# cnuns/Com-MARL

Measured on AMD Instinct MI355X. Metric: env-steps/sec (whole node), PredatorPrey M=10 N=4, 4096 envs at 1/2/4/8 GPUs, higher is better.
Workload: dtype f32

## Files before the change

### com-marl_amd/_lib.py

```python
import ctypes as C
import os

HERE = os.path.dirname(os.path.abspath(__file__))
LIB_PATH = os.environ.get("COMMARL_LIB") or os.path.join(HERE, "libcommarl_hip.so")

CM_PP, CM_CO = 0, 1
PACK_F32, PACK_F16, PACK_WAVE, PACK_CHECK, PACK_ALL = 1, 2, 4, 8, 15
CHANNELS = {"FC": 0, "FL": 1, "IID": 2, "GE": 3}
RNG_PHILOX, RNG_TAPE = 0, 1
ENT_ADD, ENT_SOFTPLUS, ENT_STOP_GRAD = 1, 2, 4
EPI_COLS, SUM_COLS = 9, 12
COMM_COLS, EPC_COLS = 4, 4
ATTN_COLS, EPA_COLS = 6, 6
LISTEN_COLS, EPL_COLS = 6, 6


class EnvCfg(C.Structure):
    _fields_ = [(n, C.c_int32) for n in (
        "scenario", "n_envs", "n_agents", "n_preys", "grid", "rsen", "load", "max_steps", "max_path_length",
        "n_hops", "rcom", "channel", "obst_hard", "add_clock", "rng_mode", "env_id_offset")] + [
        ("ploss", C.c_float), ("pgb", C.c_float), ("pbg", C.c_float), ("ge_flags", C.c_int32)] + [
        (n, C.c_double) for n in ("capture_reward", "step_cost", "move_cost", "penalty", "lazy_penalty",
                                  "revisit_penalty", "final_reward")] + [("seed", C.c_uint64)]

# ... 197 lines not shown
    "cm_comm_means": (C.c_int, [C.c_int32, C.c_int32, C.c_void_p, C.c_void_p, C.c_void_p]),
    "cm_episode_curves": (C.c_int, [C.c_int32, C.c_int32, C.c_int32, C.c_int32, C.c_void_p, C.c_void_p, C.c_void_p, C.c_void_p,
                                    C.c_void_p, C.c_int32, C.c_int32, C.c_int32, C.c_void_p, C.c_void_p]),
    "cm_curve_means": (C.c_int, [C.c_int32, C.c_int32, C.c_int32, C.c_int32, C.c_int32, C.c_void_p, C.c_void_p, C.c_void_p]),
    "cm_comm_curves": (C.c_int, [C.c_int32, C.c_int32, C.c_int32, C.c_int32, C.c_void_p, C.c_void_p, C.c_int32, C.c_int32,
                                 C.c_int32, C.c_void_p, C.c_void_p]),
    "cm_comm_curve_means": (C.c_int, [C.c_int32, C.c_int32, C.c_int32, C.c_int32, C.c_int32, C.c_void_p, C.c_void_p, C.c_void_p]),
    "cm_attn_stats": (C.c_int, [C.c_int32, C.c_int32, C.c_int32, C.c_void_p, C.c_int64, C.c_void_p, C.c_int64, C.c_void_p, C.c_int64,
                                C.c_void_p, C.c_void_p]),
    "cm_episode_attn": (C.c_int, [C.c_int32, C.c_int32, C.c_int32, C.c_int32, C.c_void_p, C.c_void_p, C.c_int32, C.c_int32,
                                  C.c_int32, C.c_int32, C.c_void_p, C.c_void_p]),
    "cm_attn_means": (C.c_int, [C.c_int32, C.c_int32, C.c_void_p, C.c_void_p, C.c_void_p]),
    "cm_attn_curves": (C.c_int, [C.c_int32, C.c_int32, C.c_int32, C.c_int32, C.c_void_p, C.c_void_p, C.c_int32, C.c_int32,
                                 C.c_int32, C.c_void_p, C.c_void_p]),
    "cm_attn_curve_means": (C.c_int, [C.c_int32, C.c_int32, C.c_int32, C.c_int32, C.c_int32, C.c_void_p, C.c_void_p, C.c_void_p]),
    "cm_listen_stats": (C.c_int, [C.c_int32, C.c_int32, C.c_int32, C.c_void_p, C.c_int64, C.c_void_p, C.c_int64, C.c_void_p, C.c_int64,
                                  C.c_void_p, C.c_void_p]),
    "cm_episode_listen": (C.c_int, [C.c_int32, C.c_int32, C.c_int32, C.c_void_p, C.c_void_p, C.c_int32, C.c_int32, C.c_int32,
                                    C.c_int32, C.c_void_p, C.c_void_p]),
    "cm_listen_means": (C.c_int, [C.c_int32, C.c_int32, C.c_void_p, C.c_void_p, C.c_void_p]),
    "cm_listen_curves": (C.c_int, [C.c_int32, C.c_int32, C.c_int32, C.c_void_p, C.c_void_p, C.c_int32, C.c_int32, C.c_int32,
                                   C.c_void_p, C.c_void_p]),
    "cm_listen_curve_means": (C.c_int, [C.c_int32, C.c_int32, C.c_int32, C.c_int32, C.c_void_p, C.c_void_p, C.c_void_p]),
    "cm_chunk_tail": (C.c_int, [C.c_void_p, C.c_uint32, C.c_void_p, C.c_void_p, C.c_size_t, C.c_void_p, C.c_void_p,
                                C.c_size_t, C.c_void_p, C.c_void_p, C.c_size_t, C.c_void_p]),
    "cm_linear_act_forward": (C.c_int, [C.c_int64, C.c_int32, C.c_int32, C.c_void_p, C.c_void_p, C.c_int32, C.c_void_p,
                                        C.c_int32, C.c_void_p, C.c_void_p]),
    "cm_linear_act_backward": (C.c_int, [C.c_int64, C.c_int32, C.c_int32, C.c_void_p, C.c_void_p, C.c_int32, C.c_void_p,
                                         C.c_void_p, C.c_void_p, C.c_void_p, C.c_void_p, C.c_void_p, C.c_void_p]),
    "cm_linear_act_backward_ex": (C.c_int, [C.c_int64, C.c_int32, C.c_int32, C.c_void_p, C.c_void_p, C.c_int32, C.c_void_p,
                                            C.c_void_p, C.c_void_p, C.c_int32, C.c_void_p, C.c_void_p, C.c_void_p, C.c_void_p]),
    "cm_encoder_backward": (C.c_int, [C.c_int64, C.c_int32, C.c_void_p, C.c_void_p, C.c_void_p, C.c_void_p, C.c_void_p, C.c_void_p,
                                      C.c_void_p, C.c_void_p, C.c_void_p, C.c_void_p, C.c_void_p]),
    "cm_multi_copy_t": (C.c_int, [C.c_int32, C.c_void_p, C.c_void_p, C.c_void_p, C.c_void_p, C.c_void_p, C.c_void_p]),
    "cm_multi_adam_step": (C.c_int, [C.c_int32, C.c_void_p, C.c_void_p, C.c_void_p, C.c_void_p, C.c_void_p, C.c_void_p,
                                     C.c_float, C.c_float, C.c_float, C.c_float, C.c_float, C.c_int32, C.c_void_p]),
    "cm_gauss_nll_forward": (C.c_int, [C.c_int64, C.c_int32, C.c_void_p, C.c_void_p, C.c_void_p, C.c_float, C.c_int32, C.c_void_p, C.c_void_p,
                                       C.c_void_p]),
    "cm_gauss_nll_backward": (C.c_int, [C.c_int64, C.c_int32, C.c_void_p, C.c_void_p, C.c_void_p, C.c_float, C.c_int32, C.c_void_p, C.c_void_p,
                                        C.c_void_p, C.c_void_p, C.c_void_p]),
    "cm_adam_bias_corrections": (None, [C.c_float, C.c_float, C.c_int32, C.c_int32, C.c_void_p]),
    "cm_multi_adam_step_dev": (C.c_int, [C.c_int32, C.c_void_p, C.c_void_p, C.c_void_p, C.c_void_p, C.c_void_p, C.c_void_p,
                                         C.c_float, C.c_float, C.c_float, C.c_float, C.c_float, C.c_void_p, C.c_void_p, C.c_int32,
                                         C.c_void_p]),
    "cm_ppo_surrogate": (C.c_int, [C.c_int32, C.c_int32, C.c_int32, C.c_int32, C.c_void_p, C.c_void_p, C.c_void_p, C.c_void_p,
                                   C.c_void_p, C.c_float, C.c_float, C.c_int32, C.c_void_p, C.c_void_p, C.c_void_p, C.c_void_p]),
    "cm_entropy_gae": (C.c_int, [C.c_int32, C.c_int32, C.c_int32, C.c_int32, C.c_void_p, C.c_void_p, C.c_void_p, C.c_float,
                                 C.c_float, C.c_float, C.c_int32, C.c_void_p, C.c_void_p, C.c_void_p, C.c_void_p]),
    "cm_discount_returns": (C.c_int, [C.c_int32, C.c_int32, C.c_void_p, C.c_void_p, C.c_double, C.c_void_p,
                                      C.c_void_p]),
    "cm_gae": (C.c_int, [C.c_int32, C.c_int32, C.c_void_p, C.c_void_p, C.c_void_p, C.c_float, C.c_float, C.c_int32,
                         C.c_float, C.c_void_p, C.c_void_p]),
    "cm_linear_act_backward_det_ws_bytes": (C.c_size_t, [C.c_int64, C.c_int32, C.c_int32]),
    "cm_linear_act_backward_det": (C.c_int, [C.c_int64, C.c_int32, C.c_int32, C.c_void_p, C.c_void_p, C.c_int32, C.c_void_p,
                                             C.c_void_p, C.c_void_p, C.c_void_p, C.c_void_p, C.c_void_p, C.c_void_p, C.c_size_t,
                                             C.c_void_p]),
    "cm_linear_act_backward_ex_det": (C.c_int, [C.c_int64, C.c_int32, C.c_int32, C.c_void_p, C.c_void_p, C.c_int32, C.c_void_p,
                                                C.c_void_p, C.c_void_p, C.c_int32, C.c_void_p, C.c_void_p, C.c_void_p, C.c_void_p,
                                                C.c_size_t, C.c_void_p]),
    "cm_encoder_backward_det_ws_bytes": (C.c_size_t, [C.c_int64, C.c_int32]),
    "cm_encoder_backward_det": (C.c_int, [C.c_int64, C.c_int32, C.c_void_p, C.c_void_p, C.c_void_p, C.c_void_p, C.c_void_p, C.c_void_p,
                                          C.c_void_p, C.c_void_p, C.c_void_p, C.c_void_p, C.c_void_p, C.c_size_t, C.c_void_p]),
    "cm_masked_agg_backward_det_ws_bytes": (C.c_size_t, [C.c_int32, C.c_int32, C.c_int32]),
    "cm_masked_agg_backward_det": (C.c_int, [C.c_int32, C.c_int32, C.c_int32, C.c_void_p, C.c_void_p, C.c_void_p,
                                             C.c_int64, C.c_void_p, C.c_void_p, C.c_void_p, C.c_void_p, C.c_void_p, C.c_void_p,
                                             C.c_void_p, C.c_void_p, C.c_size_t, C.c_void_p]),
    "cm_masked_agg_backward_any_det_ws_bytes": (C.c_size_t, [C.c_int32, C.c_int32, C.c_int32]),
    "cm_masked_agg_backward_any_det": (C.c_int, [C.c_int32, C.c_int32, C.c_int32, C.c_void_p, C.c_void_p, C.c_void_p,
                                                 C.c_int64, C.c_void_p, C.c_void_p, C.c_void_p, C.c_void_p, C.c_void_p, C.c_void_p,
                                                 C.c_void_p, C.c_void_p, C.c_size_t, C.c_void_p]),
    "cm_linear_wgrad_det_ws_bytes": (C.c_size_t, [C.c_int64, C.c_int32, C.c_int32]),
    "cm_linear_wgrad_det": (C.c_int, [C.c_int64, C.c_int32, C.c_int32, C.c_void_p, C.c_void_p, C.c_void_p, C.c_void_p,
                                      C.c_void_p, C.c_size_t, C.c_void_p]),
    "cm_ppo_surrogate_det_ws_bytes": (C.c_size_t, [C.c_int32, C.c_int32]),
    "cm_ppo_surrogate_det": (C.c_int, [C.c_int32, C.c_int32, C.c_int32, C.c_int32, C.c_void_p, C.c_void_p, C.c_void_p, C.c_void_p,
                                       C.c_void_p, C.c_float, C.c_float, C.c_int32, C.c_void_p, C.c_void_p, C.c_void_p, C.c_void_p,
                                       C.c_size_t, C.c_void_p]),
    "cm_gauss_nll_forward_det_ws_bytes": (C.c_size_t, [C.c_int64]),
    "cm_gauss_nll_forward_det": (C.c_int, [C.c_int64, C.c_int32, C.c_void_p, C.c_void_p, C.c_void_p, C.c_float, C.c_int32, C.c_void_p,
                                           C.c_void_p, C.c_size_t, C.c_void_p]),
}
EXPORTED = tuple(_SIGNATURES)

_lib = None


class CommarlError(RuntimeError):
    pass


def lib():
    global _lib
    if _lib is None:
        if not os.path.exists(LIB_PATH):
            raise CommarlError(
                f"{LIB_PATH} not found: build it with `make -C com-marl_amd/csrc` (or __graft_entry__.build()). "
                "There is no CPU fallback.")
        L = C.CDLL(LIB_PATH)
        for name, (res, args) in _SIGNATURES.items():
            fn = getattr(L, name)
            fn.restype, fn.argtypes = res, args
        if L.cm_abi_version() != 3:
            raise CommarlError("libcommarl_hip.so ABI version mismatch")
        _lib = L
    return _lib


def slab(nbytes, device):
    import torch
    return torch.empty(max(1, (int(nbytes) + 3) // 4), dtype=torch.float32, device=device)


TWINS = {
    "cm_linear_act_backward": ("cm_linear_act_backward_det", "cm_linear_act_backward_det_ws_bytes"),
    "cm_linear_act_backward_ex": ("cm_linear_act_backward_ex_det", "cm_linear_act_backward_det_ws_bytes"),
    "cm_encoder_backward": ("cm_encoder_backward_det", "cm_encoder_backward_det_ws_bytes"),
    "cm_masked_agg_backward": ("cm_masked_agg_backward_det", "cm_masked_agg_backward_det_ws_bytes"),
    "cm_masked_agg_backward_r": ("cm_masked_agg_backward_det", "cm_masked_agg_backward_det_ws_bytes"),
    "cm_masked_agg_backward_any": ("cm_masked_agg_backward_any_det", "cm_masked_agg_backward_any_det_ws_bytes"),
    "cm_linear_wgrad": ("cm_linear_wgrad_det", "cm_linear_wgrad_det_ws_bytes"),
    "cm_ppo_surrogate": ("cm_ppo_surrogate_det", "cm_ppo_surrogate_det_ws_bytes"),
    "cm_gauss_nll_forward": ("cm_gauss_nll_forward_det", "cm_gauss_nll_forward_det_ws_bytes"),
}


def run(name, *args, device=None, maybe=False):
    if device is None:
        rc = getattr(lib(), name)(*args, current_stream())
    else:
        import torch
        with torch.cuda.device(device):
            rc = getattr(lib(), name)(*args, current_stream())
    if rc == 0:
        return True
    if maybe and rc == 1:
        return False
    check(rc, name)


def launch(name, args, ws_args, device=None, maybe=False):
    from . import deterministic
    if not deterministic():
        return run(name, *args, device=device, maybe=maybe)
    import torch
    twin, ws_bytes = TWINS[name]
    with torch.cuda.device(device):
        nb = getattr(lib(), ws_bytes)(*ws_args)
        n = len(_SIGNATURES[twin][1]) - 3
        return run(twin, *args[:n], ptr(slab(nb, "cuda")), nb, maybe=maybe)
# ... 56 lines not shown
```

### com-marl_amd/nets.py

```python
import ctypes as C
import math
import os
from collections import OrderedDict

import numpy as np
import torch
from torch import nn
from torch.distributions import Categorical, Normal

from . import _lib as L
from . import deterministic as _det


MAX_KERNEL_AGENTS = 128
MAX_FUSED_AGENTS = 80
MAX_FUSED_OBS = 80

class _Tanh(nn.Module):
    def forward(self, x):
        return torch.tanh(x)


class _ReLU(nn.Module):
    def forward(self, x):
# ... 284 lines not shown
            A = A * channels[:, hop]
        A = A / (A.sum(dim=-1, keepdim=True) + 1e-12)
        out = torch.matmul(A, hw)
        return torch.tanh(out + bias if bias is not None else out)
    return _MaskedAggregate.apply(attn, dist_adj, channels, hop, hw, bias)


class _ZeroPool:

    def __init__(self, params, device, extra=0):
        total = sum((p.numel() + 3) & ~3 for p in params) + extra
        self.buf = torch.zeros(total, dtype=torch.float32, device=device)
        self.off = 0

    def take(self, shape):
        n = 1
        for d in shape:
            n *= int(d)
        if self.off + n > self.buf.numel():
            return torch.zeros(*shape, dtype=torch.float32, device=self.buf.device)
        v = self.buf[self.off:self.off + n].view(*shape)
        self.off += (n + 3) & ~3
        return v


def _lin_bwd(x2, w, layout, dy2, y2, want_dx, has_bias, dy_add=None, pool=None):
    R, K = x2.shape
    O = dy2.shape[1]
    dx = torch.empty_like(x2) if want_dx else None
    dw = pool.take(w.shape) if pool is not None else torch.zeros_like(w)
    db = (pool.take((O,)) if pool is not None else torch.zeros(O, dtype=torch.float32, device=w.device)) if has_bias else None
    _linear_act_backward(R, K, O, x2, w, layout, dy2, dy_add, y2, dx, dw, db)
    return dx, dw, db


def _fused_shape_ok(net, obs):
    return (obs.is_cuda and 1 <= net._n_agents <= MAX_FUSED_AGENTS and 1 <= len(net.gcn_layers) <= 4
            and net._dec_obs_dim <= MAX_FUSED_OBS and len(net.encoder._layers) == 1 and net._default_shape
            and os.environ.get("COMMARL_FUSED_TRAIN", "1") != "0" and os.environ.get("COMMARL_POLICY_KERNEL", "")[:1] not in ("f", "v"))


def _fused_train_ok(net, obs):
    return torch.is_grad_enabled() and _fused_shape_ok(net, obs)


def _fwd_wave_ok(N, S):
    return (N == 4 and S >= int(os.environ.get("COMMARL_TRAIN_FWD_WAVE_MIN", "16384"))
            and (os.environ.get("COMMARL_POLICY_KERNEL") or "w")[0] not in "hfv")


def _forward_saved(name, wave, *args, device):
    if wave and L.run(name + "_wave", *args, device=device, maybe=True):
        return
    if not L.run(name, *args, device=device, maybe=True):
        raise L.CommarlError(f"{name}: no saved-forward instantiation for this shape (callers check _fused_shape_ok)")


class _FusedNetFn(torch.autograd.Function):

    @staticmethod
    def forward(ctx, net, obs, adj, ch, *params):
        N, Lh, d = net._n_agents, len(net.gcn_layers), net._dec_obs_dim
        S = obs.shape[0]
        R = S * N
        dev = obs.device
        policy = net._is_policy
# ... 15 lines not shown
        adj_c = None if adj is None else adj.contiguous()
        ch_c = None if ch is None else ch.contiguous()
        net._train_fwd = True
        wave = net._train_fwd_wave = _fwd_wave_ok(N, S)
        vals = () if policy else (z(S),)
        try:
            w = net._weights_struct()
            _forward_saved("cm_policy_forward_saved" if policy else "cm_critic_forward_saved", wave, C.byref(w), S, L.ptr(obs2),
                           L.ptr(adj_c), L.ptr(ch_c), L.ptr(attn), *map(L.ptr, vals), C.byref(sv), device=dev)
        finally:
            net._train_fwd = net._train_fwd_wave = False
        ctx.net, ctx.t, ctx.obs2, ctx.adj, ctx.ch, ctx.attn, ctx.policy = net, t, obs2, adj_c, ch_c, attn, policy
        ctx.names = [n for n, _ in net.named_parameters()]
        ctx.mark_non_differentiable(attn)
        out = t["out"].view(S, N, -1) if policy else t["out"].view(S, N)
        return out, attn

    @staticmethod
    def backward(ctx, d_out, _d_attn):
        net, t, obs2, adj, ch, attn = ctx.net, ctx.t, ctx.obs2, ctx.adj, ctx.ch, ctx.attn
        N, Lh = net._n_agents, len(net.gcn_layers)
        R = obs2.shape[0]
        S = R // N
        P = dict(net.named_parameters())
        g = {}
        pool = _ZeroPool(list(P.values()), obs2.device, extra=31 * 64 * len(net.gcn_layers))
        det = _det()
        if ctx.policy:
            hd = net.categorical_output_layer
            lins = [l.linear for l in hd._layers] + [hd._output_layers[0].linear]
            pre = ["categorical_output_layer._layers.%d.linear" % i for i in range(3)] + ["categorical_output_layer._output_layers.0.linear"]
            acts = [t["h"][Lh - 1], t["x1"], t["x2"], t["x3"]]
            d = d_out.reshape(R, -1).contiguous()
            for i in (3, 2, 1, 0):
                d, g[pre[i] + ".weight"], g[pre[i] + ".bias"] = _lin_bwd(acts[i], lins[i].weight, 0, d, None if i == 3 else acts[i + 1],
                                                                          True, True, pool=pool)
        else:
            mm = net.baseline_aggregator._mean_module
            l1, l2 = mm._layers[0].linear, mm._output_layers[0].linear
            pre = "baseline_aggregator._mean_module."
            d = d_out.reshape(R, 1).contiguous()
            d, g[pre + "_output_layers.0.linear.weight"], g[pre + "_output_layers.0.linear.bias"] = _lin_bwd(t["x1"], l2.weight, 0, d, None, True, True, pool=pool)
            d, g[pre + "_layers.0.linear.weight"], g[pre + "_layers.0.linear.bias"] = _lin_bwd(t["h"][Lh - 1], l1.weight, 0, d, t["x1"], True, True, pool=pool)
        e, q = t["e"], t["q"]
        d_res = d if net.residual else None
        dH, d_attn, dhin0 = d, None, None
        for l in reversed(range(Lh)):
            gl = net.gcn_layers[l]
            minus = e if (l == Lh - 1 and net.residual) else None
            da, dhw = torch.empty_like(attn), torch.empty_like(e)
            reps = 32 if (N == 4 and S > 16 * 512 and not det) else 1
            dgb = pool.take((reps, 64)) if gl.bias is not None else None
            L.launch("cm_masked_agg_backward_r", (S, N, 64, L.ptr(attn), L.ptr(adj), *_hop_channels(ch, l, N), L.ptr(t["hw"][l]),
                                                  L.ptr(t["h"][l]), L.ptr(minus), L.ptr(dH), L.ptr(da), L.ptr(dhw), L.ptr(dgb), reps),
                     (S, N, 64), device=obs2.device)
            if dgb is not None:
                dgb = dgb.sum(0) if reps > 1 else dgb[0]
            d_attn = da if d_attn is None else d_attn.add_(da)
            hin = t["h"][l - 1] if l > 0 else e
            dhin, g["gcn_layers.%d.weight" % l], _ = _lin_bwd(hin, gl.weight, 1, dhw, None, True, False, pool=pool)
            if gl.bias is not None:
                g["gcn_layers.%d.bias" % l] = dgb
            if l > 0:
                dH = dhin
            else:
                dhin0 = dhin
        if Lh == 0:
            raise L.CommarlError("fused training path needs at least one hop")
        dq, dE = torch.empty_like(q), torch.empty_like(e)
        L.run("cm_attention_backward", S, N, 64, L.ptr(q), L.ptr(e), L.ptr(attn), L.ptr(d_attn), L.ptr(d_res), L.ptr(dhin0),
              L.ptr(dq), L.ptr(dE), device=obs2.device)
        if net.attention_layer.attention_type == "general":
            deq, g["attention_layer.linear_in.weight"], _ = _lin_bwd(e, net.attention_layer.linear_in.weight, 0, dq, None, True, False, pool=pool)
        else:
            deq = dq
        enc1, enc2 = net.encoder._layers[0].linear, net.encoder._output_layers[0].linear
# ... 1033 lines not shown
```

### include/commarl.h

```cpp
#ifndef COMMARL_H
#define COMMARL_H
#include <stddef.h>
#include <stdint.h>

#ifdef __cplusplus
extern "C" {
#endif

#define CM_ABI_VERSION 3

enum { CM_PP = 0, CM_CO = 1 };
enum { CM_CH_FC = 0, CM_CH_FL = 1, CM_CH_IID = 2, CM_CH_GE = 3 };
enum { CM_RNG_PHILOX = 0, CM_RNG_TAPE = 1 };

enum {
    CM_OK = 0,
    CM_ERR_ARG = -1,
    CM_ERR_TAPE = -2,
    CM_ERR_TAPE_PREY = -3,
    CM_ERR_ACTION = -4,
    CM_ERR_LOAD = -5,
    CM_ERR_HIP = -6,
    CM_ERR_NOMEM = -7
};
// ... 372 lines not shown
                           const float *d_out, float *d_attn, float *d_hw, float *d_bias, void *stream);
int cm_masked_agg_backward_r(int32_t S, int32_t N, int32_t E, const float *attn, const float *dist_adj,
                             const float *chan, int64_t ch_stride, const float *hw, const float *out, const float *out_minus,
                             const float *d_out, float *d_attn, float *d_hw, float *d_bias, int32_t bias_replicas, void *stream);

int cm_attention_forward(int32_t S, int32_t N, int32_t E, const float *q, const float *e, float *m, void *stream);
int cm_attention_backward(int32_t S, int32_t N, int32_t E, const float *q, const float *e, const float *m,
                          const float *d_m, const float *d_e_add0, const float *d_e_add1, float *d_q, float *d_e, void *stream);

int cm_masked_agg_forward_any(int32_t S, int32_t N, int32_t E, const float *attn, const float *dist_adj,
                              const float *chan, int64_t ch_stride, const float *hw, const float *bias, float *out,
                              void *stream);
int cm_masked_agg_backward_any(int32_t S, int32_t N, int32_t E, const float *attn, const float *dist_adj,
                               const float *chan, int64_t ch_stride, const float *hw, const float *out, const float *out_minus,
                               const float *d_out, float *d_attn, float *d_hw, float *d_bias, void *stream);
int cm_attention_forward_any(int32_t S, int32_t N, int32_t E, const float *q, const float *e, float *m, void *stream);
int cm_attention_backward_any(int32_t S, int32_t N, int32_t E, const float *q, const float *e, const float *m,
                              const float *d_m, const float *d_e_add0, const float *d_e_add1, float *d_q, float *d_e, void *stream);

int cm_linear_wgrad(int64_t R, int32_t P, int32_t Q, const float *a, const float *b, float *c, float *colsum_a,
                    void *stream);

int cm_linear_act_forward(int64_t R, int32_t in_dim, int32_t out_dim, const float *x, const float *w, int32_t w_layout,
                          const float *bias, int32_t act, float *y, void *stream);
int cm_linear_act_backward(int64_t R, int32_t in_dim, int32_t out_dim, const float *x, const float *w, int32_t w_layout,
                           const float *dy, const float *dy2, const float *y, float *dx, float *dw, float *db, void *stream);
int cm_linear_act_backward_ex(int64_t R, int32_t in_dim, int32_t out_dim, const float *x, const float *w, int32_t w_layout,
                              const float *dy, const float *dy2, const float *y, int32_t act, float *dx, float *dw, float *db,
                              void *stream);

int cm_encoder_backward(int64_t R, int32_t d, const float *obs, const float *a1, const float *e, const float *w2, const float *dy,
                        const float *dy2, float *dw2, float *db2, float *dw1, float *db1, void *stream);

int cm_multi_copy_t(int32_t n, const float *const *src, float *const *dst, const int32_t *rows, const int32_t *cols,
                    const int32_t *transpose, void *stream);
#define CM_ADAM_NORM_FLOATS 65
int cm_multi_adam_step(int32_t n, float *const *params, float *const *grads, float *const *exp_avg, float *const *exp_avg_sq,
                       const int64_t *sizes, float *norm_ws, float max_norm, float lr, float beta1,
                       float beta2, float eps, int32_t step, void *stream);
void cm_adam_bias_corrections(float beta1, float beta2, int32_t first_step, int32_t n_steps, float *table);
int cm_multi_adam_step_dev(int32_t n, float *const *params, float *const *grads, float *const *exp_avg, float *const *exp_avg_sq,
                           const int64_t *sizes, float *norm_ws, float max_norm, float lr, float beta1, float beta2, float eps,
                           const float *bc_table, const int32_t *cursor, int32_t table_steps, void *stream);

#define CM_GAUSS_WS_BYTES 16
int cm_gauss_nll_forward(int64_t S, int32_t N, const float *per_agent, const float *returns, const float *log_std, float min_log_std,
                         int32_t has_min, float *out, void *ws, void *stream);
int cm_gauss_nll_backward(int64_t S, int32_t N, const float *per_agent, const float *returns, const float *log_std, float min_log_std,
                          int32_t has_min, const float *out, const float *g, float *d_per_agent, float *d_log_std, void *stream);

int cm_discount_returns(int32_t P, int32_t T, const double *rewards, const int32_t *lens, double gamma,
                        float *returns, void *stream);
int cm_gae(int32_t P, int32_t T, const float *rewards, const float *baselines, const int32_t *lens, float gamma,
           float lam, int32_t normalize, float eps, float *adv, void *stream);

#define CM_ENT_ADD 1
#define CM_ENT_SOFTPLUS 2
#define CM_ENT_STOP_GRAD 4
int cm_ppo_surrogate(int32_t P, int32_t T, int32_t N, int32_t A, const float *logits, const int32_t *actions,
                     const float *old_ll, const float *adv, const int32_t *lens, float clip, float ent_coeff,
                     int32_t add_entropy, double *total, int64_t *count, float *dlogits, void *stream);

#define CM_ENT_GAE_MAX_T 8192
int cm_entropy_gae(int32_t P, int32_t T, int32_t N, int32_t A, const float *logits, const float *rewards,
                   const float *baselines, float gamma, float lam, float ent_coeff, int32_t softplus, float *rewards_out,
                   float *entropy_out, float *adv, void *stream);

size_t cm_linear_act_backward_det_ws_bytes(int64_t R, int32_t K, int32_t O);
int cm_linear_act_backward_det(int64_t R, int32_t K, int32_t O, const float *x, const float *w, int32_t w_layout,
                               const float *dy, const float *dy2, const float *y, float *dx, float *dw, float *db,
                               void *ws, size_t ws_bytes, void *stream);
int cm_linear_act_backward_ex_det(int64_t R, int32_t K, int32_t O, const float *x, const float *w, int32_t w_layout,
                                  const float *dy, const float *dy2, const float *y, int32_t act, float *dx, float *dw, float *db,
                                  void *ws, size_t ws_bytes, void *stream);
size_t cm_encoder_backward_det_ws_bytes(int64_t R, int32_t d);
int cm_encoder_backward_det(int64_t R, int32_t d, const float *obs, const float *a1, const float *e, const float *w2, const float *dy,
                            const float *dy2, float *dw2, float *db2, float *dw1, float *db1, void *ws, size_t ws_bytes, void *stream);
size_t cm_masked_agg_backward_det_ws_bytes(int32_t S, int32_t N, int32_t E);
int cm_masked_agg_backward_det(int32_t S, int32_t N, int32_t E, const float *attn, const float *dist_adj,
                               const float *chan, int64_t ch_stride, const float *hw, const float *out, const float *out_minus,
                               const float *d_out, float *d_attn, float *d_hw, float *d_bias, void *ws, size_t ws_bytes, void *stream);
size_t cm_masked_agg_backward_any_det_ws_bytes(int32_t S, int32_t N, int32_t E);
int cm_masked_agg_backward_any_det(int32_t S, int32_t N, int32_t E, const float *attn, const float *dist_adj,
                                   const float *chan, int64_t ch_stride, const float *hw, const float *out, const float *out_minus,
                                   const float *d_out, float *d_attn, float *d_hw, float *d_bias, void *ws, size_t ws_bytes, void *stream);
size_t cm_linear_wgrad_det_ws_bytes(int64_t R, int32_t P, int32_t Q);
int cm_linear_wgrad_det(int64_t R, int32_t P, int32_t Q, const float *a, const float *b, float *c, float *colsum_a,
                        void *ws, size_t ws_bytes, void *stream);
size_t cm_ppo_surrogate_det_ws_bytes(int32_t P, int32_t T);
int cm_ppo_surrogate_det(int32_t P, int32_t T, int32_t N, int32_t A, const float *logits, const int32_t *actions,
                         const float *old_ll, const float *adv, const int32_t *lens, float clip, float ent_coeff,
                         int32_t add_entropy, double *total, int64_t *count, float *dlogits, void *ws, size_t ws_bytes, void *stream);
size_t cm_gauss_nll_forward_det_ws_bytes(int64_t S);
int cm_gauss_nll_forward_det(int64_t S, int32_t N, const float *per_agent, const float *returns, const float *log_std, float min_log_std,
                             int32_t has_min, float *out, void *ws, size_t ws_bytes, void *stream);

#ifdef __cplusplus
}
#endif
#endif
```

Before: 460.8 million.

## Fuse policy and critic head MLP backward into one MFMA kernel

Adds a single HIP kernel that runs the whole backward pass of the policy head (four linear+tanh layers) or the critic head (two layers), replacing a chain of per-layer linear-backward launches. Intermediate gradients stay in LDS as split-fp16 hi/lo planes with per-chunk power-of-two scaling, and the matmuls use f16 MFMA with a three-product split to keep near-f32 accuracy. Weight gradients are accumulated in registers across persistent row chunks, then merged atomically or through a deterministic slab reduction. This removes kernel launches and the global-memory round trips of intermediate activations' gradients, at the cost of a complex kernel restricted to specific layer widths, with a fallback to the old path otherwise.

```diff
diff --git a/com-marl_amd/_lib.py b/com-marl_amd/_lib.py
--- a/com-marl_amd/_lib.py
+++ b/com-marl_amd/_lib.py
@@ -253,6 +253,7 @@
                                             C.c_void_p, C.c_void_p, C.c_int32, C.c_void_p, C.c_void_p, C.c_void_p, C.c_void_p]),
     "cm_encoder_backward": (C.c_int, [C.c_int64, C.c_int32, C.c_void_p, C.c_void_p, C.c_void_p, C.c_void_p, C.c_void_p, C.c_void_p,
                                       C.c_void_p, C.c_void_p, C.c_void_p, C.c_void_p, C.c_void_p]),
+    "cm_head_backward": (C.c_int, [C.c_int64, C.c_int32] + [C.c_void_p] * 19),
     "cm_multi_copy_t": (C.c_int, [C.c_int32, C.c_void_p, C.c_void_p, C.c_void_p, C.c_void_p, C.c_void_p, C.c_void_p]),
     "cm_multi_adam_step": (C.c_int, [C.c_int32, C.c_void_p, C.c_void_p, C.c_void_p, C.c_void_p, C.c_void_p, C.c_void_p,
                                      C.c_float, C.c_float, C.c_float, C.c_float, C.c_float, C.c_int32, C.c_void_p]),
@@ -282,6 +283,8 @@
     "cm_encoder_backward_det_ws_bytes": (C.c_size_t, [C.c_int64, C.c_int32]),
     "cm_encoder_backward_det": (C.c_int, [C.c_int64, C.c_int32, C.c_void_p, C.c_void_p, C.c_void_p, C.c_void_p, C.c_void_p, C.c_void_p,
                                           C.c_void_p, C.c_void_p, C.c_void_p, C.c_void_p, C.c_void_p, C.c_size_t, C.c_void_p]),
+    "cm_head_backward_det_ws_bytes": (C.c_size_t, [C.c_int64, C.c_int32, C.c_int32]),
+    "cm_head_backward_det": (C.c_int, [C.c_int64, C.c_int32] + [C.c_void_p] * 19 + [C.c_size_t, C.c_void_p]),
     "cm_masked_agg_backward_det_ws_bytes": (C.c_size_t, [C.c_int32, C.c_int32, C.c_int32]),
     "cm_masked_agg_backward_det": (C.c_int, [C.c_int32, C.c_int32, C.c_int32, C.c_void_p, C.c_void_p, C.c_void_p,
                                              C.c_int64, C.c_void_p, C.c_void_p, C.c_void_p, C.c_void_p, C.c_void_p, C.c_void_p,
@@ -336,6 +339,7 @@
     "cm_linear_act_backward": ("cm_linear_act_backward_det", "cm_linear_act_backward_det_ws_bytes"),
     "cm_linear_act_backward_ex": ("cm_linear_act_backward_ex_det", "cm_linear_act_backward_det_ws_bytes"),
     "cm_encoder_backward": ("cm_encoder_backward_det", "cm_encoder_backward_det_ws_bytes"),
+    "cm_head_backward": ("cm_head_backward_det", "cm_head_backward_det_ws_bytes"),
     "cm_masked_agg_backward": ("cm_masked_agg_backward_det", "cm_masked_agg_backward_det_ws_bytes"),
     "cm_masked_agg_backward_r": ("cm_masked_agg_backward_det", "cm_masked_agg_backward_det_ws_bytes"),
     "cm_masked_agg_backward_any": ("cm_masked_agg_backward_any_det", "cm_masked_agg_backward_any_det_ws_bytes"),
diff --git a/com-marl_amd/csrc/cm_head_bwd.hip b/com-marl_amd/csrc/cm_head_bwd.hip
--- /dev/null
+++ b/com-marl_amd/csrc/cm_head_bwd.hip
@@ -0,0 +1,536 @@
+
+#include <algorithm>
+#include <cmath>
+#include <string>
+
+#include "cm_internal.h"
+
+namespace cm {
+namespace hb {
+
+constexpr int TPB = 512, NW = 8, ROWS = 64;
+constexpr int TS = ROWS + 8;
+typedef _Float16 h16;
+typedef _Float16 v8h __attribute__((ext_vector_type(8)));
+typedef _Float16 v4h __attribute__((ext_vector_type(4)));
+typedef _Float16 v2h __attribute__((ext_vector_type(2)));
+typedef float v4f __attribute__((ext_vector_type(4)));
+
+__device__ __forceinline__ void split(float y, h16 &h, h16 &l) { h = (h16)y; l = (h16)(y - (float)h); }
+
+__device__ __forceinline__ void lift_of(unsigned max_bits, float &s, float &inv) {
+    int e = (int)(max_bits >> 23);
+    e = e < 1 ? 127 : (e > 253 ? 253 : e);
+    s = __uint_as_float((unsigned)(254 - e) << 23);
+    inv = __uint_as_float((unsigned)e << 23);
+}
+
+__device__ __forceinline__ float wave_max(float m) {
+    int v = __float_as_int(m);
+    v = max(v, __builtin_amdgcn_update_dpp(0, v, 0xB1, 0xF, 0xF, false));
+    v = max(v, __builtin_amdgcn_update_dpp(0, v, 0x4E, 0xF, 0xF, false));
+    v = max(v, __builtin_amdgcn_update_dpp(0, v, 0x124, 0xF, 0xF, false));
+    v = max(v, __builtin_amdgcn_update_dpp(0, v, 0x128, 0xF, 0xF, false));
+    const int a = __builtin_amdgcn_readlane(v, 0), b = __builtin_amdgcn_readlane(v, 16);
+    const int c = __builtin_amdgcn_readlane(v, 32), d = __builtin_amdgcn_readlane(v, 48);
+    return __int_as_float(max(max(a, b), max(c, d)));
+}
+
+template <int FORM> struct Cfg;
+template <> struct Cfg<0> { static constexpr int W0 = 32, NA = 5, OMAX = 128; };
+template <> struct Cfg<1> { static constexpr int W0 = 64, NA = 1, OMAX = 64; };
+
+template <int FORM> struct Lds {
+    static constexpr int X2T = 0, X1T = FORM == 0 ? 2 * 64 * TS : 0, HT = FORM == 0 ? X1T + 2 * 128 * TS : 0;
+    static constexpr int ZT = HT + 2 * 64 * TS, ZR = ZT + 2 * 64 * TS;
+    static constexpr int WF = ZR + 2 * ROWS * (Cfg<FORM>::OMAX + 8);
+    static constexpr int HALVES = WF + (FORM == 0 ? 4 * 4 * 2 * 64 * 8 : 0);
+    static constexpr int W0F = 0, SLOTS = Cfg<FORM>::NA * Cfg<FORM>::W0, FLOATS = SLOTS + 8;
+    static constexpr size_t BYTES = (size_t)HALVES * 2 + (size_t)FLOATS * 4;
+};
+constexpr int RED_FLOATS = NW * 5 * 64 + NW * 8 + NW * 64 + 2 * 64 + 128;
+static_assert((size_t)RED_FLOATS * 4 <= (size_t)Lds<1>::HALVES * 2, "the end-of-kernel reductions fit into the planes");
+
+struct Args {
+    long R;
+    int A;
+    const float *d_out, *x3, *x2, *x1, *h;
+    const float *w3, *w2, *w1, *w0;
+    float *dx, *dw3, *db3, *dw2, *db2, *dw1, *db1, *dw0, *db0;
+    long slab_row;
+};
+
+template <int O, int K>
+__device__ __forceinline__ void load_w(const float *__restrict__ W, v8h (&wh)[O / 32], v8h (&wl)[O / 32], int ct, int c, int g) {
+#pragma unroll
+    for (int ks = 0; ks < O / 32; ++ks)
+#pragma unroll
+        for (int e = 0; e < 8; ++e) {
+            h16 hh, ll;
+            split(W[(size_t)(32 * ks + 8 * g + e) * K + 16 * ct + c], hh, ll);
+            wh[ks][e] = hh; wl[ks][e] = ll;
+        }
+}
+
+template <int W, int U>
+__device__ __forceinline__ int unit_cq(int tid, int u) { return (tid & 3) + 4 * (((tid >> 6) * U + u) % (W / 16)); }
+template <int W, int U>
+__device__ __forceinline__ int unit_rp(int tid, int u) { return ((tid & 63) >> 2) + 16 * (((tid >> 6) * U + u) / (W / 16)); }
+
+template <int W, int U>
+__device__ __forceinline__ void planes_from(h16 *T, const float4 (&v)[U][2], int tid) {
+    unsigned *Th = reinterpret_cast<unsigned *>(T), *Tl = reinterpret_cast<unsigned *>(T + W * TS);
+#pragma unroll
+    for (int u = 0; u < U; ++u) {
+        const int cq = unit_cq<W, U>(tid, u), rp = unit_rp<W, U>(tid, u);
+        const float a[4] = { v[u][0].x, v[u][0].y, v[u][0].z, v[u][0].w }, b[4] = { v[u][1].x, v[u][1].y, v[u][1].z, v[u][1].w };
+#pragma unroll
+        for (int j = 0; j < 4; ++j) {
+            h16 ah, al, bh, bl;
+            split(a[j], ah, al);
+            split(b[j], bh, bl);
+            const int at = ((4 * cq + j) * TS + 2 * rp) >> 1;
+            Th[at] = __builtin_bit_cast(unsigned, (v2h){ ah, bh });
+            Tl[at] = __builtin_bit_cast(unsigned, (v2h){ al, bl });
+        }
+    }
+}
+template <int W, int U>
+__device__ __forceinline__ void fetch_units(const float *__restrict__ X, long r0, long R, float4 (&v)[U][2], int tid) {
+#pragma unroll
+    for (int u = 0; u < U; ++u) {
+        const int cq = unit_cq<W, U>(tid, u), rp = unit_rp<W, U>(tid, u);
+#pragma unroll
+        for (int k = 0; k < 2; ++k) {
+            const long rw = r0 + 2 * rp + k, row = rw < R ? rw : R - 1;
+            v[u][k] = *reinterpret_cast<const float4 *>(X + row * W + 4 * cq);
+        }
+    }
+}
+
+template <int O, int K, bool WLDS = false>
+__device__ __forceinline__ void layer(const h16 *zT, const h16 *zR, const h16 *xT, const v8h (&wh)[O / 32], const v8h (&wl)[O / 32],
+                                      v4f (&acc)[O * K / 256 / NW], v4f (&d)[K / 32], float inv, int wave, int c, int g,
+                                      const v8h *wf = nullptr) {
+    constexpr int KT = K / 16, TPW = O * K / 256 / NW, RPW = K / 32, KS = O / 32;
+    const v4f zero = (v4f){ 0.f, 0.f, 0.f, 0.f };
+    static_assert(KT % TPW == 0, "the tiles of a wave lie in one row of tiles");
+    const int ot = wave * TPW / KT, kt0 = wave * TPW % KT;
+    v4f pw[TPW];
+#pragma unroll
+    for (int i = 0; i < TPW; ++i) pw[i] = zero;
+#pragma unroll
+    for (int ks = 0; ks < ROWS / 32; ++ks) {
+        const int za = (16 * ot + c) * TS + 32 * ks + 8 * g;
+        const v8h ah = *reinterpret_cast<const v8h *>(zT + za), al = *reinterpret_cast<const v8h *>(zT + O * TS + za);
+        v8h bh[TPW], bl[TPW];
+#pragma unroll
+        for (int i = 0; i < TPW; ++i) {
+            const int xa = (16 * (kt0 + i) + c) * TS + 32 * ks + 8 * g;
+            bh[i] = *reinterpret_cast<const v8h *>(xT + xa);
+            bl[i] = *reinterpret_cast<const v8h *>(xT + K * TS + xa);
+        }
+#pragma unroll
+        for (int i = 0; i < TPW; ++i) pw[i] = __builtin_amdgcn_mfma_f32_16x16x32_f16(ah, bl[i], pw[i], 0, 0, 0);
+#pragma unroll
+        for (int i = 0; i < TPW; ++i) pw[i] = __builtin_amdgcn_mfma_f32_16x16x32_f16(al, bh[i], pw[i], 0, 0, 0);
+#pragma unroll
+        for (int i = 0; i < TPW; ++i) pw[i] = __builtin_amdgcn_mfma_f32_16x16x32_f16(ah, bh[i], pw[i], 0, 0, 0);
+        __builtin_amdgcn_sched_barrier(0);
+    }
+#pragma unroll
+    for (int i = 0; i < TPW; ++i)
+#pragma unroll
+        for (int r = 0; r < 4; ++r) acc[i][r] = fmaf(pw[i][r], inv, acc[i][r]);
+    const int rt0 = (wave / KT) * RPW;
+    v4f pd[RPW];
+#pragma unroll
+    for (int i = 0; i < RPW; ++i) pd[i] = zero;
+#pragma unroll
+    for (int ks = 0; ks < KS; ++ks) {
+        v8h ah[RPW], al[RPW], bh, bl;
+#pragma unroll
+        for (int i = 0; i < RPW; ++i) {
+            const int za = (16 * (rt0 + i) + c) * (O + 8) + 32 * ks + 8 * g;
+            ah[i] = *reinterpret_cast<const v8h *>(zR + za);
+            al[i] = *reinterpret_cast<const v8h *>(zR + ROWS * (O + 8) + za);
+        }
+        if constexpr (WLDS) {
+            const int at = (((wave % KT) * KS + ks) * 2) * 64 + 16 * g + c;
+            bh = wf[at]; bl = wf[at + 64];
+        } else {
+            bh = wh[ks]; bl = wl[ks];
+        }
+#pragma unroll
+        for (int i = 0; i < RPW; ++i) pd[i] = __builtin_amdgcn_mfma_f32_16x16x32_f16(ah[i], bl, pd[i], 0, 0, 0);
+#pragma unroll
+        for (int i = 0; i < RPW; ++i) pd[i] = __builtin_amdgcn_mfma_f32_16x16x32_f16(al[i], bh, pd[i], 0, 0, 0);
+#pragma unroll
+        for (int i = 0; i < RPW; ++i) pd[i] = __builtin_amdgcn_mfma_f32_16x16x32_f16(ah[i], bh, pd[i], 0, 0, 0);
+        __builtin_amdgcn_sched_barrier(0);
+    }
+#pragma unroll
+    for (int i = 0; i < RPW; ++i)
+#pragma unroll
+        for (int r = 0; r < 4; ++r) d[i][r] = pd[i][r] * inv;
+}
+
+template <int K>
+__device__ __forceinline__ void through_tanh(v4f (&d)[K / 32], const h16 *xT, unsigned *slot, float &bsum, int wave, int lane, int c, int g) {
+    constexpr int KT = K / 16, RPW = K / 32;
+    const int ct = wave % KT, rt0 = (wave / KT) * RPW;
+    float m = 0.0f;
+#pragma unroll
+    for (int i = 0; i < RPW; ++i) {
+        const int at = (16 * ct + c) * TS + 16 * (rt0 + i) + 4 * g;
+        const v4h xh = *reinterpret_cast<const v4h *>(xT + at), xl = *reinterpret_cast<const v4h *>(xT + K * TS + at);
+#pragma unroll
+        for (int r = 0; r < 4; ++r) {
+            const float x = (float)xh[r] + (float)xl[r];
+            const float z = d[i][r] * fmaf(-x, x, 1.0f);
+            d[i][r] = z;
+            bsum += z;
+            m = fmaxf(m, fabsf(z));
+        }
+    }
+    m = wave_max(m);
+    if (lane == 0) atomicMax(slot, __float_as_uint(m));
+}
+
+template <int K>
+__device__ __forceinline__ void publish(const v4f (&d)[K / 32], h16 *zT, h16 *zR, float s, int wave, int c, int g) {
+    constexpr int KT = K / 16, RPW = K / 32;
+    const int ct = wave % KT, rt0 = (wave / KT) * RPW, col = 16 * ct + c;
+#pragma unroll
+    for (int i = 0; i < RPW; ++i) {
+        v4h hh, ll;
+#pragma unroll
+        for (int r = 0; r < 4; ++r) {
+            h16 a, b;
+            split(d[i][r] * s, a, b);
+            hh[r] = a; ll[r] = b;
+            const int row = 16 * (rt0 + i) + 4 * g + r;
+            zR[row * (K + 8) + col] = a;
+            zR[ROWS * (K + 8) + row * (K + 8) + col] = b;
+        }
+        const int at = col * TS + 16 * (rt0 + i) + 4 * g;
+        *reinterpret_cast<v4h *>(zT + at) = hh;
+        *reinterpret_cast<v4h *>(zT + K * TS + at) = ll;
+    }
+}
+
+template <int O, int K, bool DET>
+__device__ __forceinline__ void merge_tiles(float *DW, const v4f (&acc)[O * K / 256 / NW], int wave, int c, int g) {
+    constexpr int KT = K / 16, TPW = O * K / 256 / NW;
+#pragma unroll
+    for (int i = 0; i < TPW; ++i) {
+        const int t = wave * TPW + i, ot = t / KT, kt = t % KT;
+#pragma unroll
+        for (int r = 0; r < 4; ++r) merge_add<DET>(DW + (size_t)(16 * ot + 4 * g + r) * K + 16 * kt + c, acc[i][r]);
+    }
+}
+
+template <int FORM, bool DET>
+__global__ __launch_bounds__(TPB) void head_bwd_kernel(Args a) {
+    using CF = Cfg<FORM>;
+    using LD = Lds<FORM>;
+    constexpr int W0 = CF::W0, NA = CF::NA, NQ = W0 / 4, U0 = ROWS * NQ / TPB;
+    constexpr bool POL = FORM == 0;
+    constexpr int O0 = POL ? 128 : 64;
+    extern __shared__ __attribute__((aligned(16))) unsigned char lds_raw[];
+    h16 *hl = reinterpret_cast<h16 *>(lds_raw);
+    float *fl = reinterpret_cast<float *>(lds_raw + (size_t)LD::HALVES * 2);
+    float *w0s = fl + LD::W0F;
+    unsigned *slots = reinterpret_cast<unsigned *>(fl + LD::SLOTS);
+    h16 *x2T = hl + LD::X2T, *x1T = hl + LD::X1T, *hT = hl + LD::HT, *zT = hl + LD::ZT, *zR = hl + LD::ZR;
+    v8h *wf = reinterpret_cast<v8h *>(hl + LD::WF);
+    const int tid = threadIdx.x, wave = tid >> 6, lane = tid & 63, c = lane & 15, g = lane >> 4;
+    const long R = a.R;
+    const int A = a.A;
+    if constexpr (DET) {
+        const size_t off = (size_t)blockIdx.x * a.slab_row;
+        a.dw3 += off; a.db3 += off; a.dw0 += off; a.db0 += off;
+        if constexpr (POL) { a.dw2 += off; a.db2 += off; a.dw1 += off; a.db1 += off; }
+    }
+
+    for (int p = tid; p < NA * W0; p += TPB) w0s[p] = p < A * W0 ? a.w3[p] : 0.0f;
+    if (tid < 8) slots[tid] = 0u;
+    v8h w2h[1], w2l[1], w1h[2], w1l[2], w0h[O0 / 32], w0l[O0 / 32];
+    if constexpr (POL) {
+        load_w<32, 64>(a.w2, w2h, w2l, wave % 4, c, g);
+        load_w<64, 128>(a.w1, w1h, w1l, wave % 8, c, g);
+        if (wave < 4) {
+            load_w<O0, 64>(a.w0, w0h, w0l, wave, c, g);
+#pragma unroll
+            for (int ks = 0; ks < O0 / 32; ++ks) {
+                wf[((wave * (O0 / 32) + ks) * 2) * 64 + lane] = w0h[ks];
+                wf[((wave * (O0 / 32) + ks) * 2 + 1) * 64 + lane] = w0l[ks];
+            }
+        }
+    } else {
+        load_w<O0, 64>(a.w0, w0h, w0l, wave % 4, c, g);
+    }
+    v4f acc2[1], acc1[4], acc0[O0 * 64 / 256 / NW];
+    acc2[0] = (v4f){ 0.f, 0.f, 0.f, 0.f };
+#pragma unroll
+    for (v4f &t : acc1) t = (v4f){ 0.f, 0.f, 0.f, 0.f };
+#pragma unroll
+    for (v4f &t : acc0) t = (v4f){ 0.f, 0.f, 0.f, 0.f };
+    float aw[NA][4], ad[NA], bv[4] = { 0.f, 0.f, 0.f, 0.f }, bs1 = 0.0f, bs0 = 0.0f;
+#pragma unroll
+    for (int k = 0; k < NA; ++k) { ad[k] = 0.0f; aw[k][0] = aw[k][1] = aw[k][2] = aw[k][3] = 0.0f; }
+
+    float4 px0[U0];
+    float pd[U0][NA];
+    float4 pxa[1][2], pxb[2][2], pxc[1][2];
+    const float *X0 = POL ? a.x3 : a.x1;
+    const int q0 = tid % NQ;
+    auto fetch = [&](long chunk) {
+        const long r0 = chunk * ROWS;
+#pragma unroll
+        for (int u = 0; u < U0; ++u) {
+            const long row = r0 + (tid + u * TPB) / NQ;
+            const bool ok = row < R;
+            const long rr = ok ? row : R - 1;
+            px0[u] = *reinterpret_cast<const float4 *>(X0 + rr * W0 + 4 * q0);
+#pragma unroll
+            for (int k = 0; k < NA; ++k) pd[u][k] = (ok && k < A) ? a.d_out[rr * A + k] : 0.0f;
+        }
+        if constexpr (POL) {
+            fetch_units<64, 1>(a.x2, r0, R, pxa, tid);
+            fetch_units<128, 2>(a.x1, r0, R, pxb, tid);
+        }
+        fetch_units<64, 1>(a.h, r0, R, pxc, tid);
+    };
+
+    const long n_chunks = (R + ROWS - 1) / ROWS;
+    long ch = blockIdx.x;
+    int par = 0;
+    if (ch < n_chunks) fetch(ch);
+    __syncthreads();
+    for (; ch < n_chunks; ch += gridDim.x, par ^= 1) {
+        const int tid = thread_x(), wave = tid >> 6, lane = tid & 63, c = lane & 15, g = lane >> 4, q0 = tid % NQ;
+        const long r0 = ch * ROWS;
+        unsigned *sl = slots + 4 * par;
+        if (tid < 4) slots[4 * (par ^ 1) + tid] = 0u;
+        if constexpr (POL) {
+            planes_from<64, 1>(x2T, pxa, tid);
+            planes_from<128, 2>(x1T, pxb, tid);
+        }
+        planes_from<64, 1>(hT, pxc, tid);
+        float zv[U0][4];
+        float m = 0.0f;
+#pragma unroll
+        for (int u = 0; u < U0; ++u) {
+            const float x[4] = { px0[u].x, px0[u].y, px0[u].z, px0[u].w };
+            float dxv[4] = { 0.f, 0.f, 0.f, 0.f };
+#pragma unroll
+            for (int k = 0; k < NA; ++k) {
+                const float4 w = *reinterpret_cast<const float4 *>(w0s + k * W0 + 4 * q0);
+                const float dk = pd[u][k];
+                dxv[0] = fmaf(dk, w.x, dxv[0]); dxv[1] = fmaf(dk, w.y, dxv[1]); dxv[2] = fmaf(dk, w.z, dxv[2]); dxv[3] = fmaf(dk, w.w, dxv[3]);
+                ad[k] += dk;
+#pragma unroll
+                for (int j = 0; j < 4; ++j) aw[k][j] = fmaf(dk, x[j], aw[k][j]);
+            }
+#pragma unroll
+            for (int j = 0; j < 4; ++j) {
+                const float z = dxv[j] * fmaf(-x[j], x[j], 1.0f);
+                zv[u][j] = z;
+                bv[j] += z;
+                m = fmaxf(m, fabsf(z));
+            }
+        }
+        m = wave_max(m);
+        if (lane == 0) atomicMax(sl + 0, __float_as_uint(m));
+        const long next = ch + gridDim.x;
+        if (next < n_chunks) fetch(next);
+        __syncthreads();
+        float s, inv;
+        lift_of(sl[0], s, inv);
+#pragma unroll
+        for (int u = 0; u < U0; ++u) {
+            const int row = (tid + u * TPB) / NQ;
+            v4h hh, ll;
+#pragma unroll
+            for (int j = 0; j < 4; ++j) {
+                h16 p, q;
+                split(zv[u][j] * s, p, q);
+                hh[j] = p; ll[j] = q;
+                zT[(4 * q0 + j) * TS + row] = p;
+                zT[W0 * TS + (4 * q0 + j) * TS + row] = q;
+            }
+            *reinterpret_cast<v4h *>(zR + row * (W0 + 8) + 4 * q0) = hh;
+            *reinterpret_cast<v4h *>(zR + ROWS * (W0 + 8) + row * (W0 + 8) + 4 * q0) = ll;
+        }
+        __syncthreads();
+        if constexpr (POL) {
+            v4f d2[2];
+            layer<32, 64>(zT, zR, x2T, w2h, w2l, acc2, d2, inv, wave, c, g);
+            through_tanh<64>(d2, x2T, sl + 1, bs1, wave, lane, c, g);
+            __syncthreads();
+            lift_of(sl[1], s, inv);
+            publish<64>(d2, zT, zR, s, wave, c, g);
+            __syncthreads();
+            v4f d1[4];
+            layer<64, 128>(zT, zR, x1T, w1h, w1l, acc1, d1, inv, wave, c, g);
+            through_tanh<128>(d1, x1T, sl + 2, bs0, wave, lane, c, g);
+            __syncthreads();
+            lift_of(sl[2], s, inv);
+            publish<128>(d1, x1T, zR, s, wave, c, g);
+            __syncthreads();
+        }
+        v4f d0[2];
+        layer<O0, 64, POL>(POL ? x1T : zT, zR, hT, w0h, w0l, acc0, d0, inv, wave, c, g, wf);
+        {
+            const int ct = wave % 4, rt0 = (wave / 4) * 2;
+#pragma unroll
+            for (int i = 0; i < 2; ++i)
+#pragma unroll
+                for (int r = 0; r < 4; ++r) {
+                    const long row = r0 + 16 * (rt0 + i) + 4 * g + r;
+                    if (row < R) a.dx[row * 64 + 16 * ct + c] = d0[i][r];
+                }
+        }
+        __syncthreads();
+    }
+
+    if constexpr (POL) {
+        merge_tiles<32, 64, DET>(a.dw2, acc2, wave, c, g);
+        merge_tiles<64, 128, DET>(a.dw1, acc1, wave, c, g);
+    }
+    merge_tiles<O0, 64, DET>(a.dw0, acc0, wave, c, g);
+    float *red = reinterpret_cast<float *>(lds_raw);
+    float *rw = red, *rd = rw + NW * 5 * 64, *rb = rd + NW * 8, *r1 = rb + NW * 64, *r0s = r1 + 2 * 64;
+#pragma unroll
+    for (int o = NQ; o < 64; o <<= 1) {
+#pragma unroll
+        for (int k = 0; k < NA; ++k) {
+            ad[k] += __shfl_xor(ad[k], o);
+#pragma unroll
+            for (int j = 0; j < 4; ++j) aw[k][j] += __shfl_xor(aw[k][j], o);
+        }
+#pragma unroll
+        for (int j = 0; j < 4; ++j) bv[j] += __shfl_xor(bv[j], o);
+    }
+    if (lane < NQ) {
+#pragma unroll
+        for (int k = 0; k < NA; ++k)
+#pragma unroll
+            for (int j = 0; j < 4; ++j) rw[(wave * NA + k) * W0 + 4 * lane + j] = aw[k][j];
+#pragma unroll
+        for (int j = 0; j < 4; ++j) rb[wave * W0 + 4 * lane + j] = bv[j];
+        if (lane == 0) {
+#pragma unroll
+            for (int k = 0; k < NA; ++k) rd[wave * NA + k] = ad[k];
+        }
+    }
+    bs1 += __shfl_xor(bs1, 16); bs1 += __shfl_xor(bs1, 32);
+    bs0 += __shfl_xor(bs0, 16); bs0 += __shfl_xor(bs0, 32);
+    if constexpr (POL) {
+        if (g == 0) {
+            r1[(wave / 4) * 64 + 16 * (wave % 4) + c] = bs1;
+            r0s[16 * wave + c] = bs0;
+        }
+    }
+    __syncthreads();
+    if (tid < NA * W0) {
+        const int k = tid / W0, col = tid % W0;
+        float sum = 0.0f;
+#pragma unroll
+        for (int w = 0; w < NW; ++w) sum += rw[(w * NA + k) * W0 + col];
+        if (k < A) merge_add<DET>(a.dw3 + k * W0 + col, sum);
+    }
+    if (tid < A) {
+        float sum = 0.0f;
+#pragma unroll
+        for (int w = 0; w < NW; ++w) sum += rd[w * NA + tid];
+        merge_add<DET>(a.db3 + tid, sum);
+    }
+    if (tid < W0) {
+        float sum = 0.0f;
+#pragma unroll
+        for (int w = 0; w < NW; ++w) sum += rb[w * W0 + tid];
+        merge_add<DET>((POL ? a.db2 : a.db0) + tid, sum);
+    }
+    if constexpr (POL) {
+        if (tid < 64) merge_add<DET>(a.db1 + tid, r1[tid] + r1[64 + tid]);
+        if (tid < 128) merge_add<DET>(a.db0 + tid, r0s[tid]);
+    }
+}
+
+__host__ __device__ constexpr long slab_row(bool critic, int A) {
+    return critic ? 64 + 1 + 64 * 64 + 64 : (long)A * 32 + A + 32 * 64 + 32 + 64 * 128 + 64 + 128 * 64 + 128;
+}
+
+template <int FORM, bool DET>
+static int launch(const Args &a, hipStream_t st, int *grid) {
+    const long chunks = (a.R + ROWS - 1) / ROWS;
+    int blocks = (int)std::min<long>(std::min<long>(chunks, cu_count()), std::max<long>(1, std::lround(std::sqrt(29.0 * (double)chunks))));
+    if (DET) blocks = std::min(blocks, 512);
+    if (grid) *grid = blocks;
+    return launch_lds<&head_bwd_kernel<FORM, DET>>(dim3(blocks), dim3(TPB), Lds<FORM>::BYTES, st, a);
+}
+
+}
+
+size_t head_slab_rows(int64_t R) { return (size_t)std::min<int64_t>((R + hb::ROWS - 1) / hb::ROWS, 512); }
+
+}
+
+using namespace cm;
+
+extern "C" size_t cm_head_backward_det_ws_bytes(int64_t R, int32_t A, int32_t critic) {
+    if (R <= 0 || A < 1 || A > 5 || (critic && A != 1)) return 0;
+    return head_slab_rows(R) * (size_t)hb::slab_row(critic != 0, A) * sizeof(float);
+}
+
+template <bool DET>
+static int head_backward(const char *fn, int64_t R, int32_t A, const float *d_out, const float *x3, const float *x2, const float *x1,
+                         const float *h, const float *w3, const float *w2, const float *w1, const float *w0, float *dx, float *dw3,
+                         float *db3, float *dw2, float *db2, float *dw1, float *db1, float *dw0, float *db0, void *ws, size_t ws_bytes,
+                         void *stream) {
+    const bool critic = !x3 && !x2;
+    if (!d_out || !x1 || !h || !w3 || !w0 || !dx || !dw3 || !db3 || !dw0 || !db0) return set_error(CM_ERR_ARG, std::string(fn) + ": null argument");
+    if (!critic && (!x3 || !x2 || !w2 || !w1 || !dw2 || !db2 || !dw1 || !db1))
+        return set_error(CM_ERR_ARG, std::string(fn) + ": null argument (the policy form takes x3, x2, w2, w1 and their gradients; the critic form none of them)");
+    if (A < 1) return set_error(CM_ERR_ARG, std::string(fn) + ": A >= 1 required");
+    if (A > 5 || (critic && A != 1)) return 1;
+    const uintptr_t al = (uintptr_t)x3 | (uintptr_t)x2 | (uintptr_t)x1 | (uintptr_t)h;
+    if ((al & 15) || (((uintptr_t)d_out | (uintptr_t)dx) & 3)) return 1;
+    if (DET)
+        if (const int rc = slab_check(ws, ws_bytes, cm_head_backward_det_ws_bytes(R, A, critic), fn)) return rc;
+    if (R <= 0) return CM_OK;
+    float *const out[8] = { dw3, db3, dw0, db0, dw2, db2, dw1, db1 };
+    const int W0 = critic ? 64 : 32, O0 = critic ? 64 : 128;
+    const int len[8] = { A * W0, A, O0 * 64, O0, 32 * 64, 32, 64 * 128, 64 };
+    const int n_out = critic ? 4 : 8;
+    int off[8], at = 0;
+    for (int k = 0; k < n_out; ++k) { off[k] = at; at += len[k]; }
+    float *gp[8] = { nullptr, nullptr, nullptr, nullptr, nullptr, nullptr, nullptr, nullptr };
+    for (int k = 0; k < n_out; ++k) gp[k] = DET ? static_cast<float *>(ws) + off[k] : out[k];
+    hb::Args a{ (long)R, A, d_out, x3, x2, x1, h, w3, w2, w1, w0, dx, gp[0], gp[1], gp[4], gp[5], gp[6], gp[7], gp[2], gp[3], (long)at };
+    int grid = 0;
+    const int rc = critic ? hb::launch<1, DET>(a, (hipStream_t)stream, &grid) : hb::launch<0, DET>(a, (hipStream_t)stream, &grid);
+    if (rc || !DET) return rc;
+    for (int k0 = 0; k0 < n_out; k0 += 4) {
+        SlabSegs segs{};
+        for (int k = 0; k < 4; ++k) segs.s[k] = { out[k0 + k], off[k0 + k], len[k0 + k] };
+        segs.n_seg = 4;
+        if (const int r2 = slab_reduce(static_cast<float *>(ws), grid, at, segs, (hipStream_t)stream)) return r2;
+    }
+    return CM_OK;
+}
+
+extern "C" int cm_head_backward(int64_t R, int32_t A, const float *d_out, const float *x3, const float *x2, const float *x1, const float *h,
+                                const float *w3, const float *w2, const float *w1, const float *w0, float *dx, float *dw3, float *db3,
+                                float *dw2, float *db2, float *dw1, float *db1, float *dw0, float *db0, void *stream) {
+    return head_backward<false>(__func__, R, A, d_out, x3, x2, x1, h, w3, w2, w1, w0, dx, dw3, db3, dw2, db2, dw1, db1, dw0, db0, nullptr, 0, stream);
+}
+
+extern "C" int cm_head_backward_det(int64_t R, int32_t A, const float *d_out, const float *x3, const float *x2, const float *x1, const float *h,
+                                    const float *w3, const float *w2, const float *w1, const float *w0, float *dx, float *dw3, float *db3,
+                                    float *dw2, float *db2, float *dw1, float *db1, float *dw0, float *db0, void *ws, size_t ws_bytes,
+                                    void *stream) {
+    return head_backward<true>(__func__, R, A, d_out, x3, x2, x1, h, w3, w2, w1, w0, dx, dw3, db3, dw2, db2, dw1, db1, dw0, db0, ws, ws_bytes, stream);
+}
diff --git a/com-marl_amd/nets.py b/com-marl_amd/nets.py
--- a/com-marl_amd/nets.py
+++ b/com-marl_amd/nets.py
@@ -340,6 +340,29 @@
     db = (pool.take((O,)) if pool is not None else torch.zeros(O, dtype=torch.float32, device=w.device)) if has_bias else None
     _linear_act_backward(R, K, O, x2, w, layout, dy2, dy_add, y2, dx, dw, db)
     return dx, dw, db
+
+
+def _head_bwd(R, d_out2, acts, lins, names, g, pool):
+    widths = [tuple(l.weight.shape) for l in lins]
+    A = d_out2.shape[1]
+    if widths not in ([(128, 64), (64, 128), (32, 64), (A, 32)], [(64, 64), (1, 64)]) or any(l.bias is None for l in lins):
+        return None
+    off = pool.off
+    dx = torch.empty_like(acts[0])
+    grads = [(pool.take(l.weight.shape), pool.take(l.bias.shape)) for l in lins]
+    none2 = (None, None)
+    x3, x2 = (acts[3], acts[2]) if len(lins) == 4 else none2
+    mid = [lins[2], lins[1]] if len(lins) == 4 else [None, None]
+    gmid = [grads[2], grads[1]] if len(lins) == 4 else [none2, none2]
+    args = (R, A, L.ptr(d_out2), L.ptr(x3), L.ptr(x2), L.ptr(acts[1]), L.ptr(acts[0]), L.ptr(lins[-1].weight),
+            *(L.ptr(None if l is None else l.weight) for l in mid), L.ptr(lins[0].weight), L.ptr(dx), *map(L.ptr, grads[-1]),
+            *(L.ptr(t) for pair in gmid for t in pair), *map(L.ptr, grads[0]))
+    if not L.launch("cm_head_backward", args, (R, A, int(len(lins) == 2)), device=dx.device, maybe=True):
+        pool.off = off
+        return None
+    for nm, (dw, db) in zip(names, grads):
+        g[nm + ".weight"], g[nm + ".bias"] = dw, db
+    return dx
 
 
 def _fused_shape_ok(net, obs):
@@ -421,16 +444,23 @@
             pre = ["categorical_output_layer._layers.%d.linear" % i for i in range(3)] + ["categorical_output_layer._output_layers.0.linear"]
             acts = [t["h"][Lh - 1], t["x1"], t["x2"], t["x3"]]
             d = d_out.reshape(R, -1).contiguous()
-            for i in (3, 2, 1, 0):
+            dh = _head_bwd(R, d, acts, lins, pre, g, pool)
+            for i in (3, 2, 1, 0) if dh is None else ():
                 d, g[pre[i] + ".weight"], g[pre[i] + ".bias"] = _lin_bwd(acts[i], lins[i].weight, 0, d, None if i == 3 else acts[i + 1],
                                                                           True, True, pool=pool)
+            d = d if dh is None else dh
         else:
             mm = net.baseline_aggregator._mean_module
             l1, l2 = mm._layers[0].linear, mm._output_layers[0].linear
             pre = "baseline_aggregator._mean_module."
             d = d_out.reshape(R, 1).contiguous()
-            d, g[pre + "_output_layers.0.linear.weight"], g[pre + "_output_layers.0.linear.bias"] = _lin_bwd(t["x1"], l2.weight, 0, d, None, True, True, pool=pool)
-            d, g[pre + "_layers.0.linear.weight"], g[pre + "_layers.0.linear.bias"] = _lin_bwd(t["h"][Lh - 1], l1.weight, 0, d, t["x1"], True, True, pool=pool)
+            names = [pre + "_layers.0.linear", pre + "_output_layers.0.linear"]
+            dh = _head_bwd(R, d, [t["h"][Lh - 1], t["x1"]], [l1, l2], names, g, pool)
+            if dh is None:
+                d, g[names[1] + ".weight"], g[names[1] + ".bias"] = _lin_bwd(t["x1"], l2.weight, 0, d, None, True, True, pool=pool)
+                d, g[names[0] + ".weight"], g[names[0] + ".bias"] = _lin_bwd(t["h"][Lh - 1], l1.weight, 0, d, t["x1"], True, True, pool=pool)
+            else:
+                d = dh
         e, q = t["e"], t["q"]
         d_res = d if net.residual else None
         dH, d_attn, dhin0 = d, None, None
diff --git a/include/commarl.h b/include/commarl.h
--- a/include/commarl.h
+++ b/include/commarl.h
@@ -428,6 +428,10 @@
 int cm_encoder_backward(int64_t R, int32_t d, const float *obs, const float *a1, const float *e, const float *w2, const float *dy,
                         const float *dy2, float *dw2, float *db2, float *dw1, float *db1, void *stream);
 
+int cm_head_backward(int64_t R, int32_t A, const float *d_out, const float *x3, const float *x2, const float *x1, const float *h,
+                     const float *w3, const float *w2, const float *w1, const float *w0, float *dx, float *dw3, float *db3,
+                     float *dw2, float *db2, float *dw1, float *db1, float *dw0, float *db0, void *stream);
+
 int cm_multi_copy_t(int32_t n, const float *const *src, float *const *dst, const int32_t *rows, const int32_t *cols,
                     const int32_t *transpose, void *stream);
 #define CM_ADAM_NORM_FLOATS 65
@@ -472,6 +476,10 @@
 size_t cm_encoder_backward_det_ws_bytes(int64_t R, int32_t d);
 int cm_encoder_backward_det(int64_t R, int32_t d, const float *obs, const float *a1, const float *e, const float *w2, const float *dy,
                             const float *dy2, float *dw2, float *db2, float *dw1, float *db1, void *ws, size_t ws_bytes, void *stream);
+size_t cm_head_backward_det_ws_bytes(int64_t R, int32_t A, int32_t critic);
+int cm_head_backward_det(int64_t R, int32_t A, const float *d_out, const float *x3, const float *x2, const float *x1, const float *h,
+                         const float *w3, const float *w2, const float *w1, const float *w0, float *dx, float *dw3, float *db3,
+                         float *dw2, float *db2, float *dw1, float *db1, float *dw0, float *db0, void *ws, size_t ws_bytes, void *stream);
 size_t cm_masked_agg_backward_det_ws_bytes(int32_t S, int32_t N, int32_t E);
 int cm_masked_agg_backward_det(int32_t S, int32_t N, int32_t E, const float *attn, const float *dist_adj,
                                const float *chan, int64_t ch_stride, const float *hw, const float *out, const float *out_minus,
```

Result: no change. 458.4 million (median of 2 runs) (-0.5%).
